# OzAmram/CaloDiffusion

Hardware: AMD Instinct MI355X
Metric: sampled showers/sec (Dataset-2, 400-step DDIM) (higher is better)
Workload: dtype f32 (convs: fp32 operands as 2-term fp16 splits on the fp16 MFMA pipe, fp32 accumulate; attention/norms fp32)

## Files before the change

### calodiffusion_amd/csrc/kernels_conv_zs.hip

```cpp
#include "cd_common.h"
#include "split16.h"
#include "gn_defer.h"

#include <cstdio>
#include <cstdlib>
#include <cstring>

namespace cd {

__device__ __forceinline__ void pack_weights_f16x2_elem(size_t idx, const float* __restrict__ w, u32x4* __restrict__ wpk, int cout,
                                                        int cin, int taps, int transposed, int flip) {
  const int lane = idx & 63;
  size_t rest = idx >> 6;
  const int CT = (cout + 31) / 32;
  const int ct = rest % CT;
  rest /= CT;
  const int tap = rest % taps;
  const int ks = rest / taps;
  const int h = lane >> 5, j = lane & 31;
  const int co = ct * 32 + j;
  f32x4 v[2];
#pragma unroll
  for (int e = 0; e < 8; ++e) {
    const int ci = ks * 16 + h * 8 + e;
// ... 446 lines not shown
constexpr int Z3_COEF = 1024;
constexpr int Z3_XCH = 4 * 2048;

template <typename T>
__device__ __forceinline__ __attribute__((address_space(3))) T* z3_lds(int byte_addr) {
  return (__attribute__((address_space(3))) T*)(uintptr_t)(unsigned)byte_addr;
}

__device__ unsigned long long z3_stamp_buf[256 * 4 * 12];
__device__ __forceinline__ unsigned long long z3_stamp() {
  unsigned long long t;
  __builtin_amdgcn_sched_barrier(0);
  asm volatile("s_memtime %0\n\ts_waitcnt lgkmcnt(0)" : "=s"(t)::"memory");
  __builtin_amdgcn_sched_barrier(0);
  return t;
}

struct Z3Geo : ZsGeo {
  int XCH;
};
__device__ __forceinline__ Z3Geo z3_geo(const ConvZsArgs& a) {
  Z3Geo g;
  (ZsGeo&)g = zs_geo(a);
  if (Z3_PAD) {
    g.pitch = a.W + 1;
    g.PLB = ((g.rows * g.pitch + 1) * ZS_VB + 255) & ~255;
  }
  g.RB = ZS_ZERO + Z3_COEF;
  g.XCH = g.RB + a.NR * g.PLB;
  g.ZPART = g.XCH;
  return g;
}

template <int WV, bool ACC, int MODE, int DBG = 0, int NSL = ZS_NSL>
__device__ __forceinline__ void z3_wave(const ConvZsArgs& a, char* lds) {
  constexpr bool NORMED = (MODE & 1) != 0, HALO = (MODE & 2) != 0, SCALED = (MODE & 4) != 0;
  constexpr int KSTEP = WV & 1, TILE = WV >> 1;
  constexpr int TH = WV >> 1, RH = WV & 1;
  static_assert(ZS_TILES == 2 && TH == TILE, "a wave reduces half of the tile it multiplies; its partner (the other k-step) the other half");
  const int lane = threadIdx.x & 63, half = lane >> 5, col = lane & 31;
  const int tid = threadIdx.x;
  const int b = blockIdx.y, ct = blockIdx.z;
  unsigned long long t_begin = 0, t_loop = 0;
  if (DBG) t_begin = z3_stamp();
  const Z3Geo G = z3_geo(a);
  const int H = a.HS, W = a.W, PV = G.PV, SPV = G.SPV;
  const int NIMG = G.rows * W;
  const int nsteps = G.nsteps;
  const int chunk = G.chunk + G.strip * a.nchunk;
  float* const coef_lds = (float*)(lds + ZS_ZERO);
  float* const bias_lds = (float*)(lds + ZS_ZERO + 512);
  int* const flag_lds = (int*)(lds + ZS_ZERO + 640);

  u32x4 w1[27], w2[27];

  const int q = tid & 7, p0 = tid >> 3;
  const float* const src_b = a.in + (size_t)b * G.vox * a.ldc;
  const int src_off = (G.h0 - G.halo) * W;
  float gscale = 1.f, ginv = 1.f;
  if (SCALED) pow2_scale_for(*a.in_absmax, &gscale, &ginv);
  int srco[NSL];
  int dsto[NSL];
#pragma unroll
  for (int k = 0; k < NSL; ++k) {
    const int pi = min(p0 + 32 * k, NIMG - 1);
    int v = pi + src_off;
    v = v < 0 ? v + PV : (v >= PV ? v - PV : v);
    srco[k] = (v * a.ldc + q * 4) * 4;
    dsto[k] = (Z3_PAD ? pi + pi / W + 1 : pi) * ZS_VB + (q >> 2) * 64 + (q & 3) * 8 + G.RB;
  }
  f32x4 ld[NSL];
  static_assert(NSL == 5 || NSL == 7 || NSL == 8, "Z3_LANDED names five, seven or eight staging registers");
  constexpr int NYOUNG = 0;
  auto uniform_ptr = [](const void* p) {
    const unsigned long long v = (unsigned long long)p;
    const unsigned lo = __builtin_amdgcn_readfirstlane((unsigned)v), hi = __builtin_amdgcn_readfirstlane((unsigned)(v >> 32));
    return (const float*)(((unsigned long long)hi << 32) | lo);
  };
  auto issue = [&](int z) {
    const int zc = min(max(z, 0), a.D - 1);
    const float* src = uniform_ptr(src_b + (size_t)zc * PV * a.ldc);
#pragma unroll
    for (int k = 0; k < NSL; ++k)
      asm volatile("global_load_dwordx4 %0, %1, %2 ; zs_plane_load" : "=v"(ld[k]) : "v"(srco[k]), "s"(src) : "memory");
  };
#define Z3_LANDED(younger)                                                                                   \
  do {                                                                                                       \
    asm volatile("s_waitcnt vmcnt(%8) ; zs_landed"                                                           \
                 : "+v"(ld[0]), "+v"(ld[1]), "+v"(ld[2]), "+v"(ld[3]), "+v"(ld[4]), "+v"(ld[NSL > 5 ? 5 : 0]),  \
                   "+v"(ld[NSL > 5 ? 6 : 1]), "+v"(ld[NSL > 7 ? 7 : 2])                                       \
                 : "n"(younger)                                                                              \
                 : "memory");                                                                                \
  } while (0)
  auto convert = [&](f32x4 (&v)[NSL], int z) {
    float amax = 0.f;
    const int zz = z + a.NR;
    const int slot = a.NR == 4 ? (zz & 3) : zz - 5 * ((zz * 205) >> 10);
    const bool zero = z < 0 || z >= a.D;
    const int sbase = slot * G.PLB;
    f32x4 cf[4], cn[4];
    if (NORMED) {
#pragma unroll
      for (int e = 0; e < 4; ++e) {
        cf[e] = *z3_lds<const f32x4>(ZS_ZERO + (q * 4 + e) * 16);
        cn[e][0] = cf[e][0] * -1.4426950408889634f;
        cn[e][1] = cf[e][1] * -1.4426950408889634f;
      }
    }
    if (zero) {
#pragma unroll
      for (int k = 0; k < NSL; ++k) {
        int d = dsto[k] + sbase;
        asm volatile("" : "+v"(d));
        *z3_lds<u32x2>(d) = u32x2{0u, 0u};
        *z3_lds<u32x2>(d + 32) = u32x2{0u, 0u};
      }
      return;
    }
#pragma unroll
    for (int k = 0; k < NSL; ++k) {
      u32x2 t1, t2;
      f32x4 x = v[k];
      if (SCALED) x = x * gscale;
      if (NORMED) {
#pragma unroll
        for (int e = 0; e < 4; ++e) {
          const float t = cf[e][0] * x[e] + cf[e][1];
          const float ex = __builtin_amdgcn_exp2f(cn[e][0] * x[e] + cn[e][1]);
          x[e] = t * __builtin_amdgcn_rcpf(1.f + ex) + cf[e][2];
        }
      }
      amax = fmaxf(fmaxf(amax, fabsf(x[0])), fabsf(x[1]));
      amax = fmaxf(fmaxf(amax, fabsf(x[2])), fabsf(x[3]));
      split2(x, t1, t2);
      int d = dsto[k] + sbase;
      asm volatile("" : "+v"(d));
      *z3_lds<u32x2>(d) = t1;
      *z3_lds<u32x2>(d + 32) = t2;
    }
    if (amax > 65504.f) *flag_lds = 1;
  };

  auto need = [&](int k) {
    k = min(k, nsteps - 1);
    return min(G.v0 + k * ZS_STEP + ZS_STEP - 1, G.cend - 1) / SPV + 1;
  };
  struct { int k, vend, zlim, need; } trk;
  auto trk_init = [&](int k) {
    trk.k = k;
    trk.vend = min(G.v0 + k * ZS_STEP + ZS_STEP - 1, G.cend - 1);
    const int zv = trk.vend / SPV;
    trk.zlim = (zv + 1) * SPV;
    trk.need = zv + 1;
  };
  auto trk_next = [&]() {
    trk.k += 1;
    if (trk.k >= nsteps) return -2;
    trk.vend = min(trk.vend + ZS_STEP, G.cend - 1);
    if (trk.vend < trk.zlim) return -2;
    trk.zlim += SPV;
    trk.need += 1;
    return trk.need;
  };

  if (tid < ZS_ZERO / 4) ((float*)lds)[tid] = 0.f;
  if (Z3_PAD)
    for (int i = tid * 16; i < a.NR * G.PLB; i += 256 * 16) *z3_lds<f32x4>(G.RB + i) = f32x4{0.f, 0.f, 0.f, 0.f};
  if (tid < 32) bias_lds[tid] = a.bias ? a.bias[ct * 32 + tid] : 0.f;
  if (tid == 32) *flag_lds = 0;
  const int zstaged0 = need(0);
  const int zp0 = G.zfirst - 1;
  trk_init(0);
  int zpend = trk_next();
  if (zpend != -2) issue(zpend);
  {
    f32x4 ldp[4][NSL];
    auto fetch = [&](f32x4 (&dst)[NSL], int z) {
      const int zc = min(max(z, 0), a.D - 1);
      const char* src = (const char*)(src_b + (size_t)zc * PV * a.ldc);
#pragma unroll
      for (int k = 0; k < NSL; ++k) dst[k] = *(const f32x4*)(src + srco[k]);
    };
#pragma unroll
    for (int i = 0; i < 3; ++i) fetch(ldp[i], zp0 + i);
    if (zp0 + 3 <= zstaged0) fetch(ldp[3], zp0 + 3);
    if (NORMED) {
      if (a.defer.part) {
        char* scratch = lds + G.ZPART;
        gn_defer_to_lds(a.defer, b, (float*)scratch, scratch + a.defer.C * 16);
        if (tid < 32) *(f32x4*)(coef_lds + tid * 4) = *(const f32x4*)(scratch + (a.choff + tid) * 16);
      } else {
        if (tid < 32) *(f32x4*)(coef_lds + tid * 4) = *(const f32x4*)(a.coef + ((size_t)b * a.coef_c + tid) * 4);
      }
    }
    {
      const u32x4* wq = a.wpk + ((size_t)(KSTEP * 27) * a.CTtot + ct) * 128 + lane;
#pragma unroll
      for (int j = 0; j < 27; ++j) {
        w1[j] = wq[(size_t)j * a.CTtot * 128];
        w2[j] = wq[(size_t)j * a.CTtot * 128 + 64];
      }
    }
    __syncthreads();
#pragma unroll
    for (int i = 0; i < 3; ++i) convert(ldp[i], zp0 + i);
    if (zp0 + 3 <= zstaged0) convert(ldp[3], zp0 + 3);
  }
#pragma unroll
  for (int j = 0; j < 27; ++j) asm volatile("" : "+a"(w1[j]), "+a"(w2[j]));

  int gh, gw, po, sb;
  const int RWB = G.pitch * ZS_VB;
  const int ring_bytes = a.NR * G.PLB;
  {
    const int v = G.v0 + TILE * 32 + col;
    const int gz = v / SPV;
    const int p = v - gz * SPV;
    gh = p / W;
    gw = p - gh * W;
    po = ((gh + (HALO ? 1 : 0)) * G.pitch + gw) * ZS_VB + G.RB + KSTEP * 64 + half * 16 - (Z3_PAD ? 0 : ZS_VB);
    sb = ((gz + a.NR - 1) % a.NR) * G.PLB;
  }
  const int adv_h = ZS_STEP / W, adv_w = ZS_STEP - adv_h * W;
  const int adv_po = (adv_h * G.pitch + adv_w) * ZS_VB, plane_po = H * RWB;
  auto advance_step = [&]() {
    gw += adv_w;
    gh += adv_h;
    po += adv_po;
    if (gw >= W) { gw -= W; gh += 1; po += (G.pitch - W) * ZS_VB; }
    if (gh >= H) {
      gh -= H;
      po -= plane_po;
      sb += G.PLB;
      sb = sb == ring_bytes ? 0 : sb;
    }
  };
  int rb[1][3][3], aL[1][3][3], aR[1][3][3];
  const int W1 = W - 1;
  auto prepare = [&]() {
    {
      constexpr int t = 0;
      const int mL = gw == 0 ? 255 : -1, mR = gw == W1 ? 255 : -1;
      int ro0, ro2;
      if (HALO) {
        ro0 = -RWB;
        ro2 = RWB;
      } else {
        ro0 = gh > 0 ? -RWB : (H - 1) * RWB;
        ro2 = gh < H - 1 ? RWB : -(H - 1) * RWB;
      }
      int bz[3];
      bz[0] = sb + po;
#pragma unroll
      for (int kz = 1; kz < 3; ++kz) {
        const unsigned x = (unsigned)(sb + kz * G.PLB);
        bz[kz] = (int)min(x, x - (unsigned)ring_bytes) + po;
      }
#pragma unroll
// ... 116 lines not shown
      }
#pragma unroll
      for (int r = 0; r < 4; ++r) {
        sum[r] = sum[r] + bvv;
        s1 = s1 + sum[r];
        s2 = s2 + sum[r] * sum[r];
      }
#pragma unroll
      for (int r = 0; r < 8; ++r)
        asm volatile("global_store_dword %0, %1, %2" ::"v"(off[r]), "v"(sum[r >> 1][r & 1]), "s"(tb) : "memory");
    } else {
#pragma unroll
      for (int r = 0; r < 8; ++r) {
        if (vt + rrow8[r] < G.cend) {
          float* dst = (float*)((char*)tb + (unsigned)off[r]);
          float v = sum[r >> 1][r & 1];
          if (ACC) v += *(const float*)((const char*)dst + a.acc_delta);
          v += bv1;
          *dst = v;
          s1[r & 1] += v;
          s2[r & 1] += v * v;
        }
      }
    }
  };

  __builtin_amdgcn_s_waitcnt(0x0F70);
  zs_barrier_lds();

  unsigned long long st[8] = {0, 0, 0, 0, 0, 0, 0, 0}, t0 = 0, t1 = 0;
  auto step = [&](int s, bool first) {
    if (DBG) t0 = z3_stamp();
    if (zpend != -2) {
      if (!first) Z3_LANDED(NYOUNG);
      if (DBG) { t1 = z3_stamp(); st[0] += t1 - t0; t0 = t1; }
      convert(ld, zpend);
      if (DBG) { t1 = z3_stamp(); st[1] += t1 - t0; t0 = t1; st[6] += 1; }
    }
    if (s >= 1) reduce_store(s - 1);
    __builtin_amdgcn_sched_barrier(0);
    zpend = trk_next();
    if (zpend != -2) issue(zpend);
    __builtin_amdgcn_sched_barrier(0);
    if (DBG) { t1 = z3_stamp(); st[2] += t1 - t0; t0 = t1; }
    prepare();
    if (DBG) { t1 = z3_stamp(); st[3] += t1 - t0; t0 = t1; }
    matrix(s);
    if (DBG) { t1 = z3_stamp(); st[4] += t1 - t0; t0 = t1; }
    zs_barrier_lds();
    if (DBG) { t1 = z3_stamp(); st[5] += t1 - t0; }
  };
  if (DBG) t_loop = z3_stamp();
  step(0, true);
  for (int s = 1; s < nsteps; ++s) step(s, false);
  reduce_store(nsteps - 1);
  if (DBG && lane == 0) {
    unsigned long long* d = z3_stamp_buf + ((size_t)((blockIdx.y * gridDim.x + blockIdx.x) & 255) * 4 + WV) * 12;
    for (int i = 0; i < 7; ++i) d[i] = st[i];
    d[7] = nsteps;
    d[8] = t_loop - t_begin;
    d[9] = z3_stamp() - t_begin;
  }

  if (a.ch_part) {
    const float u1 = s1[0] + s1[1], u2 = s2[0] + s2[1];
    const float t1 = u1 + __shfl_xor(u1, 32, 64), t2 = u2 + __shfl_xor(u2, 32, 64);
    if (half == 0) {
      float* dst = a.ch_part + ((((size_t)b * gridDim.x + chunk) * 4 + WV) * a.cout + ct * 32 + col) * 2;
      dst[0] = t1;
      dst[1] = t2;
    }
  }
  if (a.status && tid == 0 && *flag_lds) atomicOr(a.status, 1);
}

template <bool ACC, int MODE, int DBG = 0, int NSL = ZS_NSL>
__global__ void __launch_bounds__(256, 1) conv_zslide_sw_f16x2_kernel(ConvZsArgs a) {
  extern __shared__ __attribute__((aligned(16))) char zs_lds[];
  switch (threadIdx.x >> 6) {
    case 0: z3_wave<0, ACC, MODE, DBG, NSL>(a, zs_lds); break;
    case 1: z3_wave<1, ACC, MODE, DBG, NSL>(a, zs_lds); break;
    case 2: z3_wave<2, ACC, MODE, DBG, NSL>(a, zs_lds); break;
    default: z3_wave<3, ACC, MODE, DBG, NSL>(a, zs_lds); break;
  }
}

void z3_launch(const ConvZsArgs& a, bool acc, dim3 grid, size_t lds, hipStream_t s) {
  const int mode = ((a.coef || a.defer.part) ? 1 : 0) | (a.HS < a.H ? 2 : 0) | (a.in_absmax ? 4 : 0);
  const int staged = (a.HS + (a.HS < a.H ? 2 : 0)) * a.W;
  const int nsl = staged > 7 * 32 ? 8 : (staged > ZS_NSL * 32 ? 7 : ZS_NSL);
#define Z3_CASE(ACCV, M, N)                                                                                                           \
  if (acc == ACCV && mode == M && nsl == N) {                                                                                         \
    static bool attr = false;                                                                                                         \
    if (!attr) {                                                                                                                      \
      CD_HIP(hipFuncSetAttribute((const void*)conv_zslide_sw_f16x2_kernel<ACCV, M, 0, N>, hipFuncAttributeMaxDynamicSharedMemorySize, \
                                 160 * 1024));                                                                                        \
      attr = true;                                                                                                                    \
    }                                                                                                                                 \
    hipLaunchKernelGGL((conv_zslide_sw_f16x2_kernel<ACCV, M, 0, N>), grid, dim3(256), lds, s, a);                                      \
    return;                                                                                                                           \
  }
  Z3_CASE(false, 0, 5) Z3_CASE(false, 1, 5) Z3_CASE(false, 2, 5) Z3_CASE(false, 3, 5) Z3_CASE(false, 4, 5) Z3_CASE(false, 6, 5)
  Z3_CASE(true, 0, 5) Z3_CASE(true, 2, 5) Z3_CASE(true, 4, 5) Z3_CASE(true, 6, 5)
  Z3_CASE(false, 0, 7) Z3_CASE(false, 1, 7) Z3_CASE(false, 2, 7) Z3_CASE(false, 3, 7) Z3_CASE(false, 4, 7) Z3_CASE(false, 6, 7)
  Z3_CASE(true, 0, 7) Z3_CASE(true, 2, 7) Z3_CASE(true, 4, 7) Z3_CASE(true, 6, 7)
  Z3_CASE(false, 0, 8) Z3_CASE(false, 1, 8) Z3_CASE(false, 2, 8) Z3_CASE(false, 3, 8) Z3_CASE(false, 4, 8) Z3_CASE(false, 6, 8)
  Z3_CASE(true, 0, 8) Z3_CASE(true, 2, 8) Z3_CASE(true, 4, 8) Z3_CASE(true, 6, 8)
#undef Z3_CASE
  CD_REQUIRE(false, "z-slide conv: no kernel instance for this combination of continuation / normalised / strip / rescaled input");
}

}

bool try_launch_conv_zslide(const float* in0, int c0, const float* in1, int c1, const void* wpk_f16x2, const float* bias, float* out,
                            int batch, int cout, const ConvGeom& g, hipStream_t s, const ConvFusion& fu) {
  static const bool no_zslide = getenv("CD_NO_ZSLIDE") != nullptr;
  static const int strip_env = getenv("CD_ZS_STRIP") ? atoi(getenv("CD_ZS_STRIP")) : 0;
  static const int dbg_env = getenv("CD_ZS_DBG") ? atoi(getenv("CD_ZS_DBG")) : 0;
  if (no_zslide) return false;
  if (!(g.kd == 3 && g.kh == 3 && g.kw == 3 && g.sz == 1 && g.sh == 1 && g.sw == 1)) return false;
  if (cout % 32 || c0 % 32 || c1 % 32) return false;
  const int H = g.in.h, W = g.in.w;
  auto ring_for = [&](int hs) { return hs * W >= 2 * ZS_STEP ? 4 : 5; };
  static const bool v1_env = getenv("CD_ZS_V1") != nullptr;
  const bool normed_in = fu.coef || fu.defer.part;
  const bool v1 = v1_env || (normed_in && !fu.act) || (normed_in && fu.in_absmax) || (normed_in && (c0 + c1) > 32);
  auto lds_for = [&](int hs) {
    const int rows = hs + (hs < H ? 2 : 0);
    const size_t ring = (size_t)ring_for(hs) * (((size_t)rows * W * ZS_VB + 255) & ~(size_t)255);
    const size_t ring3 = Z3_PAD ? (size_t)ring_for(hs) * ((((size_t)rows * (W + 1) + 1) * ZS_VB + 255) & ~(size_t)255) : ring;
    return v1 ? (size_t)ZS_ZERO + ring + ZS_PART : (size_t)ZS_ZERO + Z3_COEF + ring3 + 2 * Z3_XCH;
  };
  static const bool nsl5_env = getenv("CD_ZS_NSL5") != nullptr;
  static const int nsl_env = getenv("CD_ZS_NSL") ? atoi(getenv("CD_ZS_NSL")) : 8;
  const int max_staged = (v1 || nsl5_env) ? ZS_NSL * 32 : std::min(8, std::max(5, nsl_env)) * 32;
  int HS = 0;
  for (int hs = H; hs >= 1; --hs) {
    if (H % hs) continue;
    const int rows = hs + (hs < H ? 2 : 0);
    if (hs * W < ZS_STEP || rows * W > max_staged || lds_for(hs) > 160 * 1024) continue;
    HS = hs;
    break;
  }
  if (!HS) return false;
  if (strip_env) {
    const int hs = strip_env;
    const int rows = hs + (hs < H ? 2 : 0);
    if (hs >= 1 && H % hs == 0 && hs * W >= ZS_STEP && rows * W <= max_staged && lds_for(hs) <= 160 * 1024) HS = hs;
  }
  const int nstrip = H / HS;
  const int SPV = HS * W;
  const int64_t svox = (int64_t)g.in.d * SPV;
  if (svox < 2 * ZS_STEP) return false;
  const size_t lds = lds_for(HS);
  if (fu.defer.part) {
    CD_REQUIRE(fu.defer.C >= c0 + c1 && fu.defer.C % 4 == 0, "z-slide conv: the deferred GroupNorm must cover the input channels");
    CD_REQUIRE((size_t)fu.defer.C * 16 + (size_t)gn_defer_scratch_bytes(fu.defer.C) <= (size_t)(v1 ? ZS_PART : 2 * Z3_XCH),
               "z-slide conv: the GroupNorm fold's scratch does not fit the exchange region");
  }
  CD_REQUIRE(lds <= 160 * 1024 && (int64_t)batch * (H / HS) <= 65535 * 64, "z-slide conv: launch geometry out of range");
  const int CTtot = cout / 32;
  int best = 1;
  double best_eff = 0.0;
  const int max_chunks = (int)(svox / (2 * ZS_STEP));
  for (int n = 1; n <= max_chunks && n <= 64; ++n) {
    const int64_t cv = ((svox + n - 1) / n + ZS_STEP - 1) / ZS_STEP * ZS_STEP;
    const int nc = (int)((svox + cv - 1) / cv);
    if (nc != n) continue;
    const int64_t total = (int64_t)batch * nstrip * nc * CTtot;
    const int64_t rounds = (total + 255) / 256;
    const double planes = (double)cv / SPV;
    const double eff = (double)total / (rounds * 256.0) * planes / (planes + 2.5);
    if (eff > best_eff * 1.0001) { best_eff = eff; best = n; }
  }
  int nchunk = best;
#ifdef CD_ZS_EXPERIMENTS
  if (getenv("CD_ZS_NCHUNK")) nchunk = atoi(getenv("CD_ZS_NCHUNK"));
#endif
  const int CV = (int)(((svox + nchunk - 1) / nchunk + ZS_STEP - 1) / ZS_STEP * ZS_STEP);
  static bool attr_set = false;
  if (!attr_set) {
    CD_HIP(hipFuncSetAttribute((const void*)conv_zslide_f16x2_kernel<false>, hipFuncAttributeMaxDynamicSharedMemorySize, 160 * 1024));
    CD_HIP(hipFuncSetAttribute((const void*)conv_zslide_f16x2_kernel<true>, hipFuncAttributeMaxDynamicSharedMemorySize, 160 * 1024));
    attr_set = true;
  }
  const int nblk = (c0 + c1) / 32;
  for (int kb = 0; kb < nblk; ++kb) {
    ConvZsArgs a;
    const int ch = kb * 32;
    if (ch < c0) { a.in = in0 + ch; a.ldc = c0; }
    else { a.in = in1 + (ch - c0); a.ldc = c1; }
    a.coef = fu.coef ? fu.coef + (size_t)ch * 4 : nullptr;
    a.coef_c = c0 + c1;
    a.defer = fu.defer;
    a.choff = ch;
    a.in_absmax = fu.in_absmax;
    a.act = fu.act;
    a.wpk = (const u32x4*)wpk_f16x2 + (size_t)(kb * 2) * 27 * CTtot * 128;
    a.CTtot = CTtot;
    a.bias = kb == 0 ? bias : nullptr;
    const bool add0 = kb == 0 && fu.add_src && !bias;
    a.acc_delta = add0 ? (long long)((const char*)fu.add_src - (const char*)out) : 0;
    a.out = out;
    a.cout = cout;
    a.ch_part = kb == nblk - 1 ? fu.ch_part : nullptr;
    a.D = g.in.d; a.H = g.in.h; a.W = g.in.w; a.HS = HS; a.NR = ring_for(HS);
    a.nchunk = nchunk; a.CV = CV;
    a.status = fu.status;
    a.dbg = dbg_env;
    const dim3 grid((unsigned)(nstrip * nchunk), (unsigned)batch, (unsigned)CTtot);
#ifdef CD_ZS_EXPERIMENTS
    if (kb == 0 && a.dbg == 2048 && !v1) {
      const bool normed = a.coef || a.defer.part;
      CD_REQUIRE(!a.in_absmax && a.HS == a.H, "CD_ZS_DBG=2048: whole planes, unscaled input");
      if (normed) {
        CD_HIP(hipFuncSetAttribute((const void*)conv_zslide_sw_f16x2_kernel<false, 1, 1>, hipFuncAttributeMaxDynamicSharedMemorySize, 160 * 1024));
        hipLaunchKernelGGL((conv_zslide_sw_f16x2_kernel<false, 1, 1>), grid, dim3(256), lds, s, a);
      } else {
        CD_HIP(hipFuncSetAttribute((const void*)conv_zslide_sw_f16x2_kernel<false, 0, 1>, hipFuncAttributeMaxDynamicSharedMemorySize, 160 * 1024));
        hipLaunchKernelGGL((conv_zslide_sw_f16x2_kernel<false, 0, 1>), grid, dim3(256), lds, s, a);
      }
      CD_HIP(hipGetLastError());
      static int nlaunch = 0;
      if (++nlaunch == 10) {
        CD_HIP(hipDeviceSynchronize());
        static unsigned long long h[256 * 4 * 12];
        CD_HIP(hipMemcpyFromSymbol(h, HIP_SYMBOL(z3_stamp_buf), sizeof h));
        for (int wg : {0, 100, 255})
          for (int w = 0; w < 4; ++w) {
            const unsigned long long* d = h + ((size_t)wg * 4 + w) * 12;
            const double n = (double)d[7], nc = d[6] ? (double)d[6] : 1.;
            std::fprintf(stderr, "[z3 stamps] wg %3d wave %d: per step: load wait %5.0f (per convert %5.0f)  convert %5.0f (per convert %5.0f)  issue+reduce %5.0f  prepare %5.0f  matrix %5.0f  barrier %5.0f   (%llu converts in %llu steps)  prologue %llu  kernel %llu cycles\n",
                         wg, w, d[0] / n, d[0] / nc, d[1] / n, d[1] / nc, d[2] / n, d[3] / n, d[4] / n, d[5] / n, d[6], d[7], d[8], d[9]);
          }
      }
      continue;
    }
#define ZS_DBG_CASE(D)                                                                                                     \
  case D:                                                                                                                  \
    CD_HIP(hipFuncSetAttribute((const void*)conv_zslide_f16x2_kernel<false, D>, hipFuncAttributeMaxDynamicSharedMemorySize, \
                               160 * 1024));                                                                               \
    hipLaunchKernelGGL((conv_zslide_f16x2_kernel<false, D>), grid, dim3(512), lds, s, a);                                   \
    break;
    if (kb == 0 && a.dbg && v1) {
      switch (a.dbg) {
        ZS_DBG_CASE(2) ZS_DBG_CASE(4) ZS_DBG_CASE(6) ZS_DBG_CASE(22) ZS_DBG_CASE(38) ZS_DBG_CASE(70)
        default: CD_REQUIRE(false, "CD_ZS_DBG: not an instantiated experiment");
      }
      CD_HIP(hipGetLastError());
      continue;
    }
#endif
    if (v1) {
      if (kb == 0 && !add0) hipLaunchKernelGGL(conv_zslide_f16x2_kernel<false>, grid, dim3(512), lds, s, a);
      else hipLaunchKernelGGL(conv_zslide_f16x2_kernel<true>, grid, dim3(512), lds, s, a);
    } else {
      z3_launch(a, kb != 0 || add0, grid, lds, s);
    }
    CD_HIP(hipGetLastError());
  }
  if (fu.add_src && !bias && fu.add_done) *fu.add_done = 1;
  if (fu.units) *fu.units = nstrip * nchunk * 4;
  return true;
}

}
```

### calodiffusion_amd/build.py

```python
from __future__ import annotations

import os
import subprocess
import sys
from concurrent.futures import ThreadPoolExecutor

HERE = os.path.dirname(os.path.abspath(__file__))
CSRC = os.path.join(HERE, "csrc")
LIBDIR = os.path.join(HERE, "lib")
TAG = os.environ.get("CD_BUILD_TAG", "")
LIB = os.path.join(LIBDIR, f"libcalodiff_hip{'_' + TAG if TAG else ''}.so")
SOURCES = ["kernels_conv.hip", "kernels_conv_zs.hip", "kernels_attn.hip", "kernels_conv_small.hip", "kernels_deep.hip", "kernels_wgrad16.hip", "kernels_norm_attn.hip", "kernels_misc.hip", "kernels_mlp.hip", "kernels_mlp_train.hip", "kernels_bwd.hip", "profiler.hip", "plan.hip",
           "forward.hip", "sampler.hip", "train.hip", "ops.hip", "misc_abi.hip"]
HIPCC = os.environ.get("HIPCC", "/opt/rocm/bin/hipcc")
FLAGS = ["--offload-arch=gfx950", "-O3", "-std=c++17", "-fPIC", "-fno-gpu-rdc", "-Wall", "-Wno-unused-function", "-Wno-unused-value"]
FLAGS += os.environ.get("CD_EXTRA_HIPCC_FLAGS", "").split()
FILE_FLAGS = {"kernels_conv_zs.hip": ["-mllvm", "-amdgpu-mfma-vgpr-form"]}


def _file_digest(paths, extra: str = "") -> str:
    import hashlib
    h = hashlib.sha256(extra.encode())
    for f in paths:
        h.update(os.path.basename(f).encode())
        h.update(open(f, "rb").read())
    return h.hexdigest()


def _read(path: str):
    try:
        return open(path).read().strip()
    except OSError:
        return None


def build_all(force: bool = False, verbose: bool = True) -> str:
    os.makedirs(LIBDIR, exist_ok=True)
    objdir = os.path.join(LIBDIR, "obj" + ("_" + TAG if TAG else ""))
    os.makedirs(objdir, exist_ok=True)
    inc = os.path.join(os.path.dirname(HERE), "include")
    headers = sorted(os.path.join(CSRC, f) for f in os.listdir(CSRC) if f.endswith((".h", ".inc")))
    headers += sorted(os.path.join(inc, f) for f in os.listdir(inc) if f.endswith(".h"))
    jobs = []
    objs = []
    for src in SOURCES:
# ... 52 lines not shown
```

### calodiffusion_amd/csrc/cd_common.h

```cpp
#pragma once
#include <hip/hip_runtime.h>
#include <stdint.h>
#include <stddef.h>
#include <string>

typedef float f32x4 __attribute__((ext_vector_type(4)));
typedef float f32x16 __attribute__((ext_vector_type(16)));

namespace cd {

void set_error(const std::string& msg);
struct Fail {
  int code;
  std::string msg;
};
#define CD_HIP(expr)                                                                                  \
  do {                                                                                                \
    hipError_t _e = (expr);                                                                           \
    if (_e != hipSuccess)                                                                             \
      throw cd::Fail{-2, std::string(#expr) + ": " + hipGetErrorString(_e)};                          \
  } while (0)
#define CD_REQUIRE(cond, msg)                                                                         \
  do {                                                                                                \
    if (!(cond)) throw cd::Fail{-1, std::string(msg)};                                                \
// ... 102 lines not shown
void launch_pack_weights_bf16x3(const float* w_torch, void* wpk, int cout, int cin, int taps, hipStream_t s,
                                bool transposed = false, bool flip = false);
void launch_pack_weights_f16x2(const float* w_torch, void* wpk, int cout, int cin, int taps, hipStream_t s,
                               bool transposed = false, bool flip = false);
inline void launch_pack_weights_split16(const float* w_torch, void* wpk, int cout, int cin, int taps, hipStream_t s,
                                        bool transposed = false, bool flip = false) {
  launch_pack_weights_bf16x3(w_torch, wpk, cout, cin, taps, s, transposed, flip);
  launch_pack_weights_f16x2(w_torch, (char*)wpk + packed_bf16x3_bytes(cin, cout, taps), cout, cin, taps, s, transposed, flip);
}

void launch_pack_weights(const float* w_torch, float* wpk, int cout, int cin, int taps, bool transposed, hipStream_t s,
                         bool flip = false);
void launch_pack_init_weights(const float* w_torch, float* wpk, int cout, int cin, hipStream_t s);
struct PackJob {
  const float* src;
  float* raw;
  float* pk;
  void* bf3;
  void* f16;
  int cout, cin, taps;
  int kind;
  int tr, flip;
  unsigned long long numel, n_pk, n_bf3, n_f16;
};
void launch_pack_jobs(const PackJob* d_jobs, int njobs, hipStream_t s);
void launch_pack_jobs_f16x2(const PackJob* d_jobs, int njobs, hipStream_t s);

void launch_conv_mfma(const float* in0, int c0, const float* in1, int c1, const float* wpk, const float* bias, float* out,
                      int batch, int cout, const ConvGeom& g, hipStream_t s, const ConvFusion& fu = ConvFusion());
bool try_launch_conv_zslide(const float* in0, int c0, const float* in1, int c1, const void* wpk_f16x2, const float* bias, float* out,
                            int batch, int cout, const ConvGeom& g, hipStream_t s, const ConvFusion& fu);
bool try_launch_conv_small(const float* in0, int c0, const float* in1, int c1, const void* wpk_f16x2, const float* bias, float* out,
                           int batch, int cout, const ConvGeom& g, hipStream_t s, const ConvFusion& fu);
void launch_conv_transpose_mfma(const float* in, int cin, const float* wpk, const float* bias, float* out, int batch,
                                int cout, Dims3 din, Dims3 dout, int kz, int sz, hipStream_t s,
                                const void* wpk_f16x2 = nullptr, int* status = nullptr, const unsigned* in_absmax = nullptr);

enum A_Prologue { A_NONE = 0, A_AFFINE = 1, A_SOFTMAX32 = 2, A_EXPNORM = 3 };
struct PointwiseArgs {
  const float* in0 = nullptr;
  int ld0 = 0, off0 = 0, c0 = 0;
  const float* in1 = nullptr;
  int ld1 = 0, c1 = 0;
  const float* wpk = nullptr;
  int64_t w_batch_stride = 0;
  const float* bias = nullptr;
  const float* residual = nullptr;
  float* out = nullptr;
  int batch = 0, cout = 0;
  int64_t vox = 0;
  int prologue = A_NONE;
  const float* coef = nullptr;
  int out_ld = 0, out_off = 0;
  float* ch_part = nullptr;
  const float* gn_res = nullptr;
  GnDefer gn_defer;
  const void* wpk16 = nullptr;
  int* status = nullptr;
};
inline int pointwise_units(int64_t vox) { return (int)((vox + 127) / 128); }
void launch_pointwise(const PointwiseArgs& a, hipStream_t s);

struct InitConvArgs {
  const float* x = nullptr;
  int cx = 0;
  int cin = 0;
// ... 359 lines not shown
```

### calodiffusion_amd/csrc/kernels_conv.hip

```cpp
#include "cd_common.h"
#include "split16.h"
#include "gn_defer.h"
#include <cstdio>
#include <cstdlib>
#include <cstring>
#include <algorithm>
#include <map>
#include <string>
#include <vector>

namespace cd {

static int g_conv_precision = -1;
static thread_local int tl_conv_precision_override = -1;
void set_conv_precision_override(int p) { tl_conv_precision_override = p; }
int conv_precision() {
  if (tl_conv_precision_override >= 0) return tl_conv_precision_override;
  if (g_conv_precision < 0) {
    const char* e = getenv("CD_CONV_PRECISION");
    g_conv_precision = !e ? PREC_F16X2 : (!strcmp(e, "f32") ? PREC_F32 : (!strcmp(e, "bf16x3") ? PREC_BF16X3 : PREC_F16X2));
  }
  return g_conv_precision;
}
void set_conv_precision(int p) { g_conv_precision = p; }
// ... 1588 lines not shown
  const int pick = autotune(key, (int)cand.size(), [&](int i) { launch(cand[i].nt, cand[i].vt, cand[i].ct); }, s);
  const Cand& c = cand[pick < 0 ? 0 : pick];
  return launch(c.nt, c.vt, c.ct);
}

void launch_conv_mfma(const float* in0, int c0, const float* in1, int c1, const float* wpk, const float* bias, float* out,
                      int batch, int cout, const ConvGeom& g, hipStream_t s, const ConvFusion& fu_in) {
  CD_REQUIRE((!fu_in.coef && !fu_in.defer.part) || c1 == 0, "conv: a fused input normalisation needs a single (non-concatenated) source");
  if (fu_in.units) *fu_in.units = 0;
  CD_REQUIRE(c0 % 32 == 0 && c1 % 32 == 0 && c0 > 0, "conv: channel counts must be multiples of 32");
  CD_REQUIRE(cout % 32 == 0, "conv: output channels must be a multiple of 32");
  CD_REQUIRE(g.kw <= 4, "conv: r kernel extent > 4 unsupported");
  const int CTtot = cout / 32;
  int CT = CTtot <= 3 ? CTtot : 2;
  CD_REQUIRE(CTtot % CT == 0, "conv: unsupported output channel count");
  char cat[128];
  std::snprintf(cat, sizeof cat, "conv%dx%dx%d_s%d C%d->%d @%dx%dx%d", g.kd, g.kh, g.kw, g.sh, c0 + c1, cout, g.in.d, g.in.h, g.in.w);
  const double taps = (double)g.kd * g.kh * g.kw;
  prof::Scope scope(cat, s, 2.0 * taps * (c0 + c1) * cout * (double)g.out.vox() * batch,
                    4.0 * batch * ((double)g.in.vox() * (c0 + c1) + (double)g.out.vox() * cout));
  ConvFusion fu = fu_in;
  auto materialise = [&]() {
    if (!fu.defer.part) return;
    if (fu.defer.coef_out) fu.coef_buf = fu.defer.coef_out;
    CD_REQUIRE(fu.coef_buf, "conv: deferred normalisation needs a coefficient buffer for kernels without the prologue");
    launch_gn_finalize(fu.defer.part, fu.defer.units, fu.defer.gamma, fu.defer.beta, fu.defer.add, fu.defer.add_ld, fu.coef_buf, batch,
                       fu.defer.C, fu.defer.groups, fu.defer.vox, s, fu.defer.stat_out);
    fu.coef = fu.coef_buf;
    fu.defer = GnDefer();
  };
  {
    const bool want_f32 = conv_precision() == PREC_F32, want_bf16x3 = conv_precision() == PREC_BF16X3;
    if (fu.wpk_bf16x3 && !want_f32 && !want_bf16x3 &&
        try_launch_conv_zslide(in0, c0, in1, c1, (const char*)fu.wpk_bf16x3 + packed_bf16x3_bytes(c0 + c1, cout, g.kd * g.kh * g.kw),
                               bias, out, batch, cout, g, s, fu))
      return;
    if (fu.wpk_bf16x3 && !want_f32 && !want_bf16x3 &&
        try_launch_conv_small(in0, c0, in1, c1, (const char*)fu.wpk_bf16x3 + packed_bf16x3_bytes(c0 + c1, cout, g.kd * g.kh * g.kw),
                              bias, out, batch, cout, g, s, fu))
      return;
    if (fu.wpk_bf16x3 && !want_f32 && !want_bf16x3 &&
        try_launch_conv3_flat(in0, c0, in1, c1, (const char*)fu.wpk_bf16x3 + packed_bf16x3_bytes(c0 + c1, cout, g.kd * g.kh * g.kw), bias,
                              out, batch, cout, g, s, fu, 2))
      return;
    materialise();
    if (fu.wpk_bf16x3 && !want_f32 && try_launch_conv3_flat(in0, c0, in1, c1, fu.wpk_bf16x3, bias, out, batch, cout, g, s, fu, 3))
      return;
    if (try_launch_conv3_flat(in0, c0, in1, c1, wpk, bias, out, batch, cout, g, s, fu, 0)) return;
  }
  {
    const bool want_f32 = conv_precision() == PREC_F32;
    if (fu.wpk_bf16x3 && !want_f32) {
      const bool f16_ok = conv_precision() == PREC_F16X2 && !fu.in_absmax;
      for (int pass = f16_ok ? 0 : 1; pass < 2; ++pass) {
      const bool f16 = pass == 0;
      const std::vector<ConvTile> cand3 = conv_tile_candidates(g, batch, CT, 14, f16 ? 80 : 96);
      auto launch3 = [&](const ConvTile& t) {
        ConvTiled3Args a3;
        ConvKArgs& a = a3.k;
        a3.status = fu.status;
        a.in0 = in0; a.in1 = in1; a.c0 = c0; a.c1 = c1; a.bias = bias; a.out = out;
        a.wpk = f16 ? (const float*)((const char*)fu.wpk_bf16x3 + packed_bf16x3_bytes(c0 + c1, cout, g.kd * g.kh * g.kw))
                    : (const float*)fu.wpk_bf16x3;
        a.Din = g.in.d; a.Hin = g.in.h; a.Win = g.in.w; a.Do = g.out.d; a.Ho = g.out.h; a.Wo = g.out.w;
        a.KD = g.kd; a.KH = g.kh; a.KW = g.kw; a.SZ = g.sz; a.SH = g.sh; a.SW = g.sw;
        a.TZ = t.TZ; a.TH = t.TH; a.nTZ = (g.out.d + t.TZ - 1) / t.TZ; a.nTH = (g.out.h + t.TH - 1) / t.TH;
// ... 934 lines not shown
```

Baseline: 91.29.

## Add two-plane-per-step z-slide conv path for small 32-voxel planes

Adds a PAIR mode to the z-slide conv wave kernel for layers whose H*W plane is half a step. Each step stages, converts and advances two z-planes at once, using a six-slot ring, and skips the strip and halo machinery. It is enabled by default for 32-channel single-block inputs, with an env knob to widen or disable it. The aim is better MFMA utilisation on small-plane layers, which previously fell back to the v1 kernel or the generic strip path. The cost is more template instances and a separate ring/step bookkeeping path that has to stay correct at the z boundaries.

New measurement: 91.56 (median of 6 runs). About the same (+0.3%).

```diff
diff --git a/calodiffusion_amd/csrc/kernels_conv_zs.hip b/calodiffusion_amd/csrc/kernels_conv_zs.hip
--- a/calodiffusion_amd/csrc/kernels_conv_zs.hip
+++ b/calodiffusion_amd/csrc/kernels_conv_zs.hip
@@ -502,9 +502,12 @@
   return g;
 }
 
-template <int WV, bool ACC, int MODE, int DBG = 0, int NSL = ZS_NSL>
+template <int WV, bool ACC, int MODE, int DBG = 0, int NSL = ZS_NSL, int PPS = 1>
 __device__ __forceinline__ void z3_wave(const ConvZsArgs& a, char* lds) {
   constexpr bool NORMED = (MODE & 1) != 0, HALO = (MODE & 2) != 0, SCALED = (MODE & 4) != 0;
+  constexpr bool PAIR = PPS == 2;
+  constexpr int PNR = 6;
+  static_assert(PPS == 1 || (PAIR && NSL == 2 && !HALO && !SCALED), "two-plane steps: whole 32-voxel planes, one piece per plane");
   constexpr int KSTEP = WV & 1, TILE = WV >> 1;
   constexpr int TH = WV >> 1, RH = WV & 1;
   static_assert(ZS_TILES == 2 && TH == TILE, "a wave reduces half of the tile it multiplies; its partner (the other k-step) the other half");
@@ -533,14 +536,14 @@
   int dsto[NSL];
 #pragma unroll
   for (int k = 0; k < NSL; ++k) {
-    const int pi = min(p0 + 32 * k, NIMG - 1);
+    const int pi = PAIR ? p0 : min(p0 + 32 * k, NIMG - 1);
     int v = pi + src_off;
     v = v < 0 ? v + PV : (v >= PV ? v - PV : v);
     srco[k] = (v * a.ldc + q * 4) * 4;
     dsto[k] = (Z3_PAD ? pi + pi / W + 1 : pi) * ZS_VB + (q >> 2) * 64 + (q & 3) * 8 + G.RB;
   }
   f32x4 ld[NSL];
-  static_assert(NSL == 5 || NSL == 7 || NSL == 8, "Z3_LANDED names five, seven or eight staging registers");
+  static_assert(NSL == 2 || NSL == 5 || NSL == 7 || NSL == 8, "Z3_LANDED names two, five, seven or eight staging registers");
   constexpr int NYOUNG = 0;
   auto uniform_ptr = [](const void* p) {
     const unsigned long long v = (unsigned long long)p;
@@ -548,6 +551,15 @@
     return (const float*)(((unsigned long long)hi << 32) | lo);
   };
   auto issue = [&](int z) {
+    if constexpr (PAIR) {
+#pragma unroll
+      for (int k = 0; k < 2; ++k) {
+        const int zc = min(max(z + k, 0), a.D - 1);
+        const float* src = uniform_ptr(src_b + (size_t)zc * PV * a.ldc);
+        asm volatile("global_load_dwordx4 %0, %1, %2 ; zs_plane_load" : "=v"(ld[k]) : "v"(srco[k]), "s"(src) : "memory");
+      }
+      return;
+    }
     const int zc = min(max(z, 0), a.D - 1);
     const float* src = uniform_ptr(src_b + (size_t)zc * PV * a.ldc);
 #pragma unroll
@@ -564,6 +576,45 @@
   } while (0)
   auto convert = [&](f32x4 (&v)[NSL], int z) {
     float amax = 0.f;
+    if constexpr (PAIR) {
+      f32x4 cf[4], cn[4];
+      if (NORMED) {
+#pragma unroll
+        for (int e = 0; e < 4; ++e) {
+          cf[e] = *z3_lds<const f32x4>(ZS_ZERO + (q * 4 + e) * 16);
+          cn[e][0] = cf[e][0] * -1.4426950408889634f;
+          cn[e][1] = cf[e][1] * -1.4426950408889634f;
+        }
+      }
+#pragma unroll
+      for (int k = 0; k < 2; ++k) {
+        const int zk = z + k;
+        int d = dsto[k] + ((zk + PNR) % PNR) * G.PLB;
+        asm volatile("" : "+v"(d));
+        if (zk < 0 || zk >= a.D) {
+          *z3_lds<u32x2>(d) = u32x2{0u, 0u};
+          *z3_lds<u32x2>(d + 32) = u32x2{0u, 0u};
+          continue;
+        }
+        f32x4 x = v[k];
+        if (NORMED) {
+#pragma unroll
+          for (int e = 0; e < 4; ++e) {
+            const float t = cf[e][0] * x[e] + cf[e][1];
+            const float ex = __builtin_amdgcn_exp2f(cn[e][0] * x[e] + cn[e][1]);
+            x[e] = t * __builtin_amdgcn_rcpf(1.f + ex) + cf[e][2];
+          }
+        }
+        amax = fmaxf(fmaxf(amax, fabsf(x[0])), fabsf(x[1]));
+        amax = fmaxf(fmaxf(amax, fabsf(x[2])), fabsf(x[3]));
+        u32x2 t1, t2;
+        split2(x, t1, t2);
+        *z3_lds<u32x2>(d) = t1;
+        *z3_lds<u32x2>(d + 32) = t2;
+      }
+      if (amax > 65504.f) *flag_lds = 1;
+      return;
+    }
     const int zz = z + a.NR;
     const int slot = a.NR == 4 ? (zz & 3) : zz - 5 * ((zz * 205) >> 10);
     const bool zero = z < 0 || z >= a.D;
@@ -626,6 +677,7 @@
   auto trk_next = [&]() {
     trk.k += 1;
     if (trk.k >= nsteps) return -2;
+    if (PAIR) return G.zfirst + 2 * trk.k + 1;
     trk.vend = min(trk.vend + ZS_STEP, G.cend - 1);
     if (trk.vend < trk.zlim) return -2;
     trk.zlim += SPV;
@@ -646,14 +698,25 @@
   {
     f32x4 ldp[4][NSL];
     auto fetch = [&](f32x4 (&dst)[NSL], int z) {
+      if constexpr (PAIR) {
+#pragma unroll
+        for (int k = 0; k < 2; ++k)
+          dst[k] = *(const f32x4*)((const char*)(src_b + (size_t)min(max(z + k, 0), a.D - 1) * PV * a.ldc) + srco[k]);
+        return;
+      }
       const int zc = min(max(z, 0), a.D - 1);
       const char* src = (const char*)(src_b + (size_t)zc * PV * a.ldc);
 #pragma unroll
       for (int k = 0; k < NSL; ++k) dst[k] = *(const f32x4*)(src + srco[k]);
     };
-#pragma unroll
-    for (int i = 0; i < 3; ++i) fetch(ldp[i], zp0 + i);
-    if (zp0 + 3 <= zstaged0) fetch(ldp[3], zp0 + 3);
+    if (PAIR) {
+      fetch(ldp[0], zp0);
+      fetch(ldp[1], zp0 + 2);
+    } else {
+#pragma unroll
+      for (int i = 0; i < 3; ++i) fetch(ldp[i], zp0 + i);
+      if (zp0 + 3 <= zstaged0) fetch(ldp[3], zp0 + 3);
+    }
     if (NORMED) {
       if (a.defer.part) {
         char* scratch = lds + G.ZPART;
@@ -672,9 +735,14 @@
       }
     }
     __syncthreads();
-#pragma unroll
-    for (int i = 0; i < 3; ++i) convert(ldp[i], zp0 + i);
-    if (zp0 + 3 <= zstaged0) convert(ldp[3], zp0 + 3);
+    if (PAIR) {
+      convert(ldp[0], zp0);
+      convert(ldp[1], zp0 + 2);
+    } else {
+#pragma unroll
+      for (int i = 0; i < 3; ++i) convert(ldp[i], zp0 + i);
+      if (zp0 + 3 <= zstaged0) convert(ldp[3], zp0 + 3);
+    }
   }
 #pragma unroll
   for (int j = 0; j < 27; ++j) asm volatile("" : "+a"(w1[j]), "+a"(w2[j]));
@@ -694,6 +762,11 @@
   const int adv_h = ZS_STEP / W, adv_w = ZS_STEP - adv_h * W;
   const int adv_po = (adv_h * G.pitch + adv_w) * ZS_VB, plane_po = H * RWB;
   auto advance_step = [&]() {
+    if (PAIR) {
+      sb += 2 * G.PLB;
+      sb = sb >= ring_bytes ? sb - ring_bytes : sb;
+      return;
+    }
     gw += adv_w;
     gh += adv_h;
     po += adv_po;
@@ -876,7 +949,12 @@
   auto step = [&](int s, bool first) {
     if (DBG) t0 = z3_stamp();
     if (zpend != -2) {
-      if (!first) Z3_LANDED(NYOUNG);
+      if (!first) {
+        if constexpr (PAIR)
+          asm volatile("s_waitcnt vmcnt(%2) ; zs_landed" : "+v"(ld[0]), "+v"(ld[1]) : "n"(NYOUNG) : "memory");
+        else
+          Z3_LANDED(NYOUNG);
+      }
       if (DBG) { t1 = z3_stamp(); st[0] += t1 - t0; t0 = t1; }
       convert(ld, zpend);
       if (DBG) { t1 = z3_stamp(); st[1] += t1 - t0; t0 = t1; st[6] += 1; }
@@ -921,18 +999,20 @@
 template <bool ACC, int MODE, int DBG = 0, int NSL = ZS_NSL>
 __global__ void __launch_bounds__(256, 1) conv_zslide_sw_f16x2_kernel(ConvZsArgs a) {
   extern __shared__ __attribute__((aligned(16))) char zs_lds[];
+  constexpr int PPS = NSL == 2 ? 2 : 1;
   switch (threadIdx.x >> 6) {
-    case 0: z3_wave<0, ACC, MODE, DBG, NSL>(a, zs_lds); break;
-    case 1: z3_wave<1, ACC, MODE, DBG, NSL>(a, zs_lds); break;
-    case 2: z3_wave<2, ACC, MODE, DBG, NSL>(a, zs_lds); break;
-    default: z3_wave<3, ACC, MODE, DBG, NSL>(a, zs_lds); break;
-  }
-}
-
-void z3_launch(const ConvZsArgs& a, bool acc, dim3 grid, size_t lds, hipStream_t s) {
+    case 0: z3_wave<0, ACC, MODE, DBG, NSL, PPS>(a, zs_lds); break;
+    case 1: z3_wave<1, ACC, MODE, DBG, NSL, PPS>(a, zs_lds); break;
+    case 2: z3_wave<2, ACC, MODE, DBG, NSL, PPS>(a, zs_lds); break;
+    default: z3_wave<3, ACC, MODE, DBG, NSL, PPS>(a, zs_lds); break;
+  }
+}
+
+void z3_launch(const ConvZsArgs& a, bool acc, bool pair, dim3 grid, size_t lds, hipStream_t s) {
   const int mode = ((a.coef || a.defer.part) ? 1 : 0) | (a.HS < a.H ? 2 : 0) | (a.in_absmax ? 4 : 0);
+  if (pair) CD_REQUIRE(a.NR == 6 && a.H * a.W * 2 == ZS_STEP && a.HS == a.H && mode <= 1, "z-slide conv: not a two-plane-step launch");
   const int staged = (a.HS + (a.HS < a.H ? 2 : 0)) * a.W;
-  const int nsl = staged > 7 * 32 ? 8 : (staged > ZS_NSL * 32 ? 7 : ZS_NSL);
+  const int nsl = pair ? 2 : (staged > 7 * 32 ? 8 : (staged > ZS_NSL * 32 ? 7 : ZS_NSL));
 #define Z3_CASE(ACCV, M, N)                                                                                                           \
   if (acc == ACCV && mode == M && nsl == N) {                                                                                         \
     static bool attr = false;                                                                                                         \
@@ -950,6 +1030,7 @@
   Z3_CASE(true, 0, 7) Z3_CASE(true, 2, 7) Z3_CASE(true, 4, 7) Z3_CASE(true, 6, 7)
   Z3_CASE(false, 0, 8) Z3_CASE(false, 1, 8) Z3_CASE(false, 2, 8) Z3_CASE(false, 3, 8) Z3_CASE(false, 4, 8) Z3_CASE(false, 6, 8)
   Z3_CASE(true, 0, 8) Z3_CASE(true, 2, 8) Z3_CASE(true, 4, 8) Z3_CASE(true, 6, 8)
+  Z3_CASE(false, 0, 2) Z3_CASE(false, 1, 2) Z3_CASE(true, 0, 2) Z3_CASE(true, 1, 2)
 #undef Z3_CASE
   CD_REQUIRE(false, "z-slide conv: no kernel instance for this combination of continuation / normalised / strip / rescaled input");
 }
@@ -965,10 +1046,13 @@
   if (!(g.kd == 3 && g.kh == 3 && g.kw == 3 && g.sz == 1 && g.sh == 1 && g.sw == 1)) return false;
   if (cout % 32 || c0 % 32 || c1 % 32) return false;
   const int H = g.in.h, W = g.in.w;
-  auto ring_for = [&](int hs) { return hs * W >= 2 * ZS_STEP ? 4 : 5; };
   static const bool v1_env = getenv("CD_ZS_V1") != nullptr;
   const bool normed_in = fu.coef || fu.defer.part;
-  const bool v1 = v1_env || (normed_in && !fu.act) || (normed_in && fu.in_absmax) || (normed_in && (c0 + c1) > 32);
+  static const int pair_env = getenv("CD_ZS_PAIR") ? atoi(getenv("CD_ZS_PAIR")) : 1;
+  const bool pair = pair_env > 0 && H * W * 2 == ZS_STEP && !v1_env && !fu.in_absmax && (!normed_in || fu.act) &&
+                    (pair_env > 1 || (c1 == 0 && c0 == 32));
+  auto ring_for = [&](int hs) { return pair ? 6 : (hs * W >= 2 * ZS_STEP ? 4 : 5); };
+  const bool v1 = !pair && (v1_env || (normed_in && !fu.act) || (normed_in && fu.in_absmax) || (normed_in && (c0 + c1) > 32));
   auto lds_for = [&](int hs) {
     const int rows = hs + (hs < H ? 2 : 0);
     const size_t ring = (size_t)ring_for(hs) * (((size_t)rows * W * ZS_VB + 255) & ~(size_t)255);
@@ -978,8 +1062,8 @@
   static const bool nsl5_env = getenv("CD_ZS_NSL5") != nullptr;
   static const int nsl_env = getenv("CD_ZS_NSL") ? atoi(getenv("CD_ZS_NSL")) : 8;
   const int max_staged = (v1 || nsl5_env) ? ZS_NSL * 32 : std::min(8, std::max(5, nsl_env)) * 32;
-  int HS = 0;
-  for (int hs = H; hs >= 1; --hs) {
+  int HS = pair ? H : 0;
+  for (int hs = H; hs >= 1 && !pair; --hs) {
     if (H % hs) continue;
     const int rows = hs + (hs < H ? 2 : 0);
     if (hs * W < ZS_STEP || rows * W > max_staged || lds_for(hs) > 160 * 1024) continue;
@@ -987,7 +1071,7 @@
     break;
   }
   if (!HS) return false;
-  if (strip_env) {
+  if (strip_env && !pair) {
     const int hs = strip_env;
     const int rows = hs + (hs < H ? 2 : 0);
     if (hs >= 1 && H % hs == 0 && hs * W >= ZS_STEP && rows * W <= max_staged && lds_for(hs) <= 160 * 1024) HS = hs;
@@ -1054,7 +1138,7 @@
     a.dbg = dbg_env;
     const dim3 grid((unsigned)(nstrip * nchunk), (unsigned)batch, (unsigned)CTtot);
 #ifdef CD_ZS_EXPERIMENTS
-    if (kb == 0 && a.dbg == 2048 && !v1) {
+    if (kb == 0 && a.dbg == 2048 && !v1 && !pair) {
       const bool normed = a.coef || a.defer.part;
       CD_REQUIRE(!a.in_absmax && a.HS == a.H, "CD_ZS_DBG=2048: whole planes, unscaled input");
       if (normed) {
@@ -1099,7 +1183,7 @@
       if (kb == 0 && !add0) hipLaunchKernelGGL(conv_zslide_f16x2_kernel<false>, grid, dim3(512), lds, s, a);
       else hipLaunchKernelGGL(conv_zslide_f16x2_kernel<true>, grid, dim3(512), lds, s, a);
     } else {
-      z3_launch(a, kb != 0 || add0, grid, lds, s);
+      z3_launch(a, kb != 0 || add0, pair, grid, lds, s);
     }
     CD_HIP(hipGetLastError());
   }
```

## Add streaming persistent kernel for strided 3x4x4 downsample convs

Applied to the files above, without the earlier changes.

Adds a dedicated persistent kernel for the 32->32 channel 3x4x4 stride-2 downsampling conv. Each block walks a contiguous range of output z-planes and keeps a ring of split-fp16 input planes in LDS, so each input plane is loaded and converted once rather than re-read per output tap. Weights stay in registers and the next plane's global loads are issued before the MFMA work on the current plane. The cost is one block per CU (launch_bounds 1), an LDS cross-wave reduction per plane, and periodic boundary handling in H.

Result: no change. 87.06 before, 87.11 after, median of 6 (+0.1%).

```diff
diff --git a/calodiffusion_amd/build.py b/calodiffusion_amd/build.py
--- a/calodiffusion_amd/build.py
+++ b/calodiffusion_amd/build.py
@@ -10,7 +10,7 @@
 LIBDIR = os.path.join(HERE, "lib")
 TAG = os.environ.get("CD_BUILD_TAG", "")
 LIB = os.path.join(LIBDIR, f"libcalodiff_hip{'_' + TAG if TAG else ''}.so")
-SOURCES = ["kernels_conv.hip", "kernels_conv_zs.hip", "kernels_attn.hip", "kernels_conv_small.hip", "kernels_deep.hip", "kernels_wgrad16.hip", "kernels_norm_attn.hip", "kernels_misc.hip", "kernels_mlp.hip", "kernels_mlp_train.hip", "kernels_bwd.hip", "profiler.hip", "plan.hip",
+SOURCES = ["kernels_conv.hip", "kernels_conv_zs.hip", "kernels_attn.hip", "kernels_conv_small.hip", "kernels_resample.hip", "kernels_deep.hip", "kernels_wgrad16.hip", "kernels_norm_attn.hip", "kernels_misc.hip", "kernels_mlp.hip", "kernels_mlp_train.hip", "kernels_bwd.hip", "profiler.hip", "plan.hip",
            "forward.hip", "sampler.hip", "train.hip", "ops.hip", "misc_abi.hip"]
 HIPCC = os.environ.get("HIPCC", "/opt/rocm/bin/hipcc")
 FLAGS = ["--offload-arch=gfx950", "-O3", "-std=c++17", "-fPIC", "-fno-gpu-rdc", "-Wall", "-Wno-unused-function", "-Wno-unused-value"]
diff --git a/calodiffusion_amd/csrc/cd_common.h b/calodiffusion_amd/csrc/cd_common.h
--- a/calodiffusion_amd/csrc/cd_common.h
+++ b/calodiffusion_amd/csrc/cd_common.h
@@ -158,6 +158,8 @@
                             int batch, int cout, const ConvGeom& g, hipStream_t s, const ConvFusion& fu);
 bool try_launch_conv_small(const float* in0, int c0, const float* in1, int c1, const void* wpk_f16x2, const float* bias, float* out,
                            int batch, int cout, const ConvGeom& g, hipStream_t s, const ConvFusion& fu);
+bool try_launch_resample_down(const float* in0, int c0, const float* in1, int c1, const void* wpk_f16x2, const float* bias, float* out,
+                              int batch, int cout, const ConvGeom& g, hipStream_t s, const ConvFusion& fu);
 void launch_conv_transpose_mfma(const float* in, int cin, const float* wpk, const float* bias, float* out, int batch,
                                 int cout, Dims3 din, Dims3 dout, int kz, int sz, hipStream_t s,
                                 const void* wpk_f16x2 = nullptr, int* status = nullptr, const unsigned* in_absmax = nullptr);
diff --git a/calodiffusion_amd/csrc/kernels_conv.hip b/calodiffusion_amd/csrc/kernels_conv.hip
--- a/calodiffusion_amd/csrc/kernels_conv.hip
+++ b/calodiffusion_amd/csrc/kernels_conv.hip
@@ -1644,6 +1644,10 @@
   {
     const bool want_f32 = conv_precision() == PREC_F32, want_bf16x3 = conv_precision() == PREC_BF16X3;
     if (fu.wpk_bf16x3 && !want_f32 && !want_bf16x3 &&
+        try_launch_resample_down(in0, c0, in1, c1, (const char*)fu.wpk_bf16x3 + packed_bf16x3_bytes(c0 + c1, cout, g.kd * g.kh * g.kw),
+                                 bias, out, batch, cout, g, s, fu))
+      return;
+    if (fu.wpk_bf16x3 && !want_f32 && !want_bf16x3 &&
         try_launch_conv_zslide(in0, c0, in1, c1, (const char*)fu.wpk_bf16x3 + packed_bf16x3_bytes(c0 + c1, cout, g.kd * g.kh * g.kw),
                                bias, out, batch, cout, g, s, fu))
       return;
diff --git a/calodiffusion_amd/csrc/kernels_resample.hip b/calodiffusion_amd/csrc/kernels_resample.hip
--- /dev/null
+++ b/calodiffusion_amd/csrc/kernels_resample.hip
@@ -0,0 +1,204 @@
+#include "cd_common.h"
+#include "split16.h"
+
+#include <cstdio>
+#include <cstdlib>
+
+namespace cd {
+
+namespace {
+
+constexpr int kRsVB = 144;
+constexpr int kRsMaxPlane = 160;
+constexpr int kRsThreads = 512;
+constexpr int kRsQPT = (kRsMaxPlane * 8 + kRsThreads - 1) / kRsThreads;
+constexpr int kRsSlots = 4;
+
+struct ResampleDownArgs {
+  const float* in;
+  const u32x4* wpk;
+  const float* bias;
+  float* out;
+  int D, H, W, Ho, Wo, Do;
+  int planes;
+  int* status;
+  const unsigned* in_absmax;
+};
+
+template <int SZ>
+__global__ void __launch_bounds__(kRsThreads, 1) resample_down_f16x2_kernel(ResampleDownArgs a) {
+  extern __shared__ __attribute__((aligned(16))) float lds[];
+  char* ldsb = (char*)lds;
+  constexpr int KW = 4;
+  const int tid = threadIdx.x, lane = tid & 63, wave = tid >> 6;
+  const int half = lane >> 5, col = lane & 31;
+  const int HW = a.H * a.W, HWo = a.Ho * a.Wo;
+  const int nq = HW * 8;
+  const int slot_bytes = HW * kRsVB;
+  const int zero_off = kRsSlots * slot_bytes;
+  float* red = (float*)(ldsb + ((zero_off + kRsVB + 15) & ~15));
+
+  const int q0 = (int)(((long long)blockIdx.x * a.planes) / gridDim.x);
+  const int q1 = (int)(((long long)(blockIdx.x + 1) * a.planes) / gridDim.x);
+  if (tid < kRsVB / 4) ((float*)(ldsb + zero_off))[tid] = 0.f;
+
+  const int kh = wave >> 1, ks = wave & 1;
+  u32x4 wr[3][KW][2];
+#pragma unroll
+  for (int kz = 0; kz < 3; ++kz)
+#pragma unroll
+    for (int kw = 0; kw < KW; ++kw)
+#pragma unroll
+      for (int t = 0; t < 2; ++t) wr[kz][kw][t] = a.wpk[((size_t)ks * 48 + kz * 16 + kh * KW + kw) * 128 + t * 64 + lane];
+
+  int rel[KW];
+  {
+    const bool valid = col < HWo;
+    const int oh = valid ? col / a.Wo : 0, ow = valid ? col - oh * a.Wo : 0;
+    int ih = 2 * oh + kh - 1;
+    ih = ih < 0 ? ih + a.H : (ih >= a.H ? ih - a.H : ih);
+    ih = ih >= a.H ? ih - a.H : ih;
+#pragma unroll
+    for (int kw = 0; kw < KW; ++kw) {
+      const int iw = 2 * ow + kw - 1;
+      rel[kw] = valid && iw >= 0 && iw < a.W ? (ih * a.W + iw) * kRsVB : -1;
+    }
+  }
+
+  float gscale = 1.f, ginv = 1.f;
+  if (a.in_absmax) pow2_scale_for(*a.in_absmax, &gscale, &ginv);
+  float amax = 0.f;
+  f32x4 bv = {0.f, 0.f, 0.f, 0.f};
+  if (a.bias) {
+    const float* bp = a.bias + (tid & 7) * 4;
+    bv = f32x4{bp[0], bp[1], bp[2], bp[3]};
+  }
+
+  f32x4 sv[2][kRsQPT];
+  bool sok[2] = {false, false};
+  auto load_plane = [&](int j, int b, int iz) {
+    sok[j] = iz >= 0 && iz < a.D;
+    const f32x4* src = (const f32x4*)(a.in + ((size_t)b * a.D + min(max(iz, 0), a.D - 1)) * HW * 32);
+#pragma unroll
+    for (int k = 0; k < kRsQPT; ++k) sv[j][k] = src[min(tid + k * kRsThreads, nq - 1)];
+  };
+  auto store_plane = [&](int j, int iz) {
+    char* base = ldsb + ((iz + 1) & (kRsSlots - 1)) * slot_bytes;
+#pragma unroll
+    for (int k = 0; k < kRsQPT; ++k) {
+      const int i = tid + k * kRsThreads;
+      if (i < nq) {
+        const f32x4 vs = sok[j] ? sv[j][k] * gscale : f32x4{0.f, 0.f, 0.f, 0.f};
+        amax = fmaxf(amax, fmaxf(fmaxf(fabsf(vs[0]), fabsf(vs[1])), fmaxf(fabsf(vs[2]), fabsf(vs[3]))));
+        u32x2 t1, t2;
+        split2(vs, t1, t2);
+        char* d = base + (i >> 3) * kRsVB + (i & 7) * 8;
+        *(u32x2*)d = t1;
+        *(u32x2*)(d + 64) = t2;
+      }
+    }
+  };
+
+  if (q0 < q1) {
+    const int b = q0 / a.Do, oz = q0 - b * a.Do;
+    load_plane(0, b, SZ * oz - 1);
+    store_plane(0, SZ * oz - 1);
+    load_plane(0, b, SZ * oz);
+    load_plane(1, b, SZ * oz + 1);
+    store_plane(0, SZ * oz);
+    store_plane(1, SZ * oz + 1);
+  }
+  __syncthreads();
+
+  for (int q = q0; q < q1; ++q) {
+    const int b = q / a.Do, oz = q - b * a.Do;
+    const bool has_next = q + 1 < q1;
+    const int nb = oz + 1 == a.Do ? b + 1 : b, noz = oz + 1 == a.Do ? 0 : oz + 1;
+    const bool need0 = has_next && (SZ == 2 || noz == 0);
+    if (need0) load_plane(0, nb, SZ * noz);
+    if (has_next) load_plane(1, nb, SZ * noz + 1);
+
+    f32x16 acc, accB;
+#pragma unroll
+    for (int r = 0; r < 16; ++r) acc[r] = accB[r] = 0.f;
+#pragma unroll
+    for (int kz = 0; kz < 3; ++kz) {
+      const int sb = ((SZ * oz + kz) & (kRsSlots - 1)) * slot_bytes;
+#pragma unroll
+      for (int kw = 0; kw < KW; ++kw) {
+        const char* p = ldsb + (rel[kw] >= 0 ? sb + rel[kw] : zero_off) + ks * 32 + half * 16;
+        const u32x4 a1 = *(const u32x4*)p, a2 = *(const u32x4*)(p + 64);
+        acc = MFMA_F16(a1, wr[kz][kw][0], acc);
+        accB = MFMA_F16(a1, wr[kz][kw][1], accB);
+        accB = MFMA_F16(a2, wr[kz][kw][0], accB);
+      }
+    }
+#pragma unroll
+    for (int r = 0; r < 16; ++r) red[(wave * 32 + (r & 3) + 8 * (r >> 2) + 4 * half) * 32 + col] = acc[r] + accB[r] * (1.f / 2048.f);
+    __syncthreads();
+    if (tid * 4 < HWo * 32) {
+      const f32x4* rp = (const f32x4*)red + tid;
+      f32x4 v = rp[0];
+#pragma unroll
+      for (int w = 1; w < kRsThreads / 64; ++w) v += rp[w * 256];
+      v = v * ginv + bv;
+      *(f32x4*)(a.out + (size_t)q * HWo * 32 + tid * 4) = v;
+    }
+    if (has_next) {
+      if (noz == 0) {
+        u32x4* z = (u32x4*)ldsb;
+        for (int i = tid; i < slot_bytes / 16; i += kRsThreads) z[i] = u32x4{0u, 0u, 0u, 0u};
+      }
+      if (need0) store_plane(0, SZ * noz);
+      store_plane(1, SZ * noz + 1);
+    }
+    __syncthreads();
+  }
+  if (a.status && amax > 65504.f) atomicOr(a.status, 1);
+}
+
+template <int SZ>
+void launch_resample_down_inst(const ResampleDownArgs& a, int grid, size_t lds, hipStream_t s) {
+  static bool attr_set = false;
+  if (!attr_set) {
+    CD_HIP(hipFuncSetAttribute((const void*)resample_down_f16x2_kernel<SZ>, hipFuncAttributeMaxDynamicSharedMemorySize, 160 * 1024));
+    attr_set = true;
+  }
+  hipLaunchKernelGGL((resample_down_f16x2_kernel<SZ>), dim3((unsigned)grid), dim3(kRsThreads), lds, s, a);
+  CD_HIP(hipGetLastError());
+}
+
+int cu_count() {
+  static int n = 0;
+  if (!n) {
+    int dev = 0;
+    CD_HIP(hipGetDevice(&dev));
+    CD_HIP(hipDeviceGetAttribute(&n, hipDeviceAttributeMultiprocessorCount, dev));
+    if (n <= 0) n = 1;
+  }
+  return n;
+}
+
+}
+
+bool try_launch_resample_down(const float* in0, int c0, const float* in1, int c1, const void* wpk_f16x2, const float* bias, float* out,
+                              int batch, int cout, const ConvGeom& g, hipStream_t s, const ConvFusion& fu) {
+  if (getenv("CD_NO_RESAMPLE_STREAM") || !wpk_f16x2) return false;
+  if (g.kd != 3 || g.kh != 4 || g.kw != 4 || g.sh != 2 || g.sw != 2 || (g.sz != 1 && g.sz != 2)) return false;
+  if (c0 != 32 || c1 != 0 || in1 || cout != 32) return false;
+  if (fu.coef || fu.defer.part || fu.ch_part || fu.add_src || fu.gn_out.gamma) return false;
+  const int HW = g.in.h * g.in.w, HWo = g.out.h * g.out.w;
+  if (HW > kRsMaxPlane || HWo > 32 || g.out.d < 1) return false;
+  ResampleDownArgs a;
+  a.in = in0; a.wpk = (const u32x4*)wpk_f16x2; a.bias = bias; a.out = out;
+  a.D = g.in.d; a.H = g.in.h; a.W = g.in.w; a.Ho = g.out.h; a.Wo = g.out.w; a.Do = g.out.d;
+  a.planes = batch * g.out.d;
+  a.status = fu.status; a.in_absmax = fu.in_absmax;
+  const size_t lds = (((size_t)kRsSlots * HW * kRsVB + kRsVB + 15) & ~(size_t)15) + (kRsThreads / 64) * 32 * 32 * 4;
+  const int grid = a.planes < cu_count() ? a.planes : cu_count();
+  if (g.sz == 2) launch_resample_down_inst<2>(a, grid, lds, s);
+  else launch_resample_down_inst<1>(a, grid, lds, s);
+  return true;
+}
+
+}
```
